# georgematheos/Gen

Measured on AMD Instinct MI355X. Metric: particle-steps/sec (whole node) + log-ML error vs CPU ref, 1M-particle SSM, higher is better.
Workload: dtype f64; 1 GPU; C2: 10-dim linear-Gaussian SSM bootstrap PF, 1048576 particles/GPU, systematic resampling at ESS<N/2, record_history=True; particles_global=1048576, d=10, resampler=systematic, parallelism=particle-dp1, transport=none, filters=46

## Files before the change

gen_amd/csrc/gh_kernels.h:

```cpp
#pragma once
#include "gh_models.h"

namespace gh {

constexpr int kBlock = 256;
constexpr int kScanItems = 4;
constexpr int kScanTile = kBlock * kScanItems;

constexpr int kTileP = 64;
__host__ __device__ __forceinline__ int64_t tbase(int64_t i, int D) { return (i >> 6) * (int64_t)(kTileP * D); }
__host__ __device__ __forceinline__ int64_t xidx(int64_t i, int k, int D) {
  const int l = (int)(i & 63);
  return tbase(i, D) + (k < (D & ~1) ? (k >> 1) * (2 * kTileP) + 2 * l + (k & 1) : (D - 1) * kTileP + l);
}
__host__ __device__ __forceinline__ int64_t slot_doubles(int64_t n, int D) {
  return ((n + kTileP - 1) / kTileP) * (int64_t)(kTileP * D);
}

struct DevScalars {
  double stats[3];
  double log_ml_est;
  double M, L, ess;
  double sM;
  uint64_t S;
  uint64_t base;
  uint64_t local;
  uint64_t o, Qs, Rs;
  double invN;
  double invS;
  int pending;
  int fire;
  int spend;
  int one;
  int error;
  unsigned ticket;
  unsigned ticket_q;
  unsigned ticket_c;
  double cM, cL, cess;
  int cfire, cerr;
  unsigned bar_gen;
  int64_t ra, rb;
  unsigned fire_streak;
};

constexpr int kErrBarrier = 7;
constexpr int kErrGenealogy = 7 | 1 << 8;
constexpr int kErrPeer = 7 | 2 << 8;

struct StepArgs {
  const double* xprev;
  int32_t* anc;
  const uint32_t* mark;
  const uint32_t* carry;
  uint32_t mark_idx;
  int mark_mode;
  int resampled;
  int buf;
  const double* remote;
  int64_t ld_remote;
  double* xout;
  double* logw;
  int64_t n;
  int64_t nvb;
  int max_only;
  int64_t lo;
  uint64_t seed;
  uint32_t t;
  int proposal;
  DevScalars* dev;
  double* pm;
  double* ps;
  double* ps2;
  double* stats_out;
  uint64_t* amax;
  int part;
  int64_t j0;
  int64_t vb_split, vb_skip;
  int64_t grid_blocks;
  double* rhist;
};

template <int CTRL, int ROW_MASK = 0xf>
__device__ __forceinline__ uint64_t dpp_u64(uint64_t v, uint64_t old) {
  const int lo = __builtin_amdgcn_update_dpp((int)(uint32_t)old, (int)(uint32_t)v, CTRL, ROW_MASK, 0xf, false);
  const int hi = __builtin_amdgcn_update_dpp((int)(uint32_t)(old >> 32), (int)(uint32_t)(v >> 32), CTRL, ROW_MASK,
                                             0xf, false);
  return ((uint64_t)(uint32_t)hi << 32) | (uint64_t)(uint32_t)lo;
}
template <int CTRL, int ROW_MASK = 0xf>
__device__ __forceinline__ double dpp_f64(double v, double old) {
  return as_f64(dpp_u64<CTRL, ROW_MASK>(as_u64(v), as_u64(old)));
}
__device__ __forceinline__ uint64_t readfirstlane_u64(uint64_t v) {
  const uint32_t lo = (uint32_t)__builtin_amdgcn_readfirstlane((int)(uint32_t)v);
  const uint32_t hi = (uint32_t)__builtin_amdgcn_readfirstlane((int)(uint32_t)(v >> 32));
  return ((uint64_t)hi << 32) | lo;
}
__device__ __forceinline__ uint64_t readlane63_u64(uint64_t v) {
  const uint32_t lo = (uint32_t)__builtin_amdgcn_readlane((int)(uint32_t)v, 63);
  const uint32_t hi = (uint32_t)__builtin_amdgcn_readlane((int)(uint32_t)(v >> 32), 63);
  return ((uint64_t)hi << 32) | lo;
}

template <int CTRL, int ROW_MASK = 0xf>
__device__ __forceinline__ uint64_t dpp_red_u64(uint64_t v) {
  const int lo = __builtin_amdgcn_mov_dpp((int)(uint32_t)v, CTRL, ROW_MASK, 0xf, true);
  const int hi = __builtin_amdgcn_mov_dpp((int)(uint32_t)(v >> 32), CTRL, ROW_MASK, 0xf, true);
  return ((uint64_t)(uint32_t)hi << 32) | (uint64_t)(uint32_t)lo;
}
template <int CTRL, int ROW_MASK = 0xf>
__device__ __forceinline__ double dpp_red_f64(double v) {
  return as_f64(dpp_red_u64<CTRL, ROW_MASK>(as_u64(v)));
}

template <class Op>
__device__ __forceinline__ double wave_reduce_f64(double v, Op op) {
  v = op(v, dpp_red_f64<0xb1>(v));
  v = op(v, dpp_red_f64<0x4e>(v));
  v = op(v, dpp_red_f64<0x114>(v));
  v = op(v, dpp_red_f64<0x118>(v));
  v = op(v, dpp_red_f64<0x142, 0xa>(v));
  v = op(v, dpp_red_f64<0x143, 0xc>(v));
  return as_f64(readlane63_u64(as_u64(v)));
}
__device__ __forceinline__ double wave_max(double v) {
  return wave_reduce_f64(v, [](double a, double b) { return fmax(a, b); });
}
__device__ __forceinline__ double wave_sum(double v) {
  return wave_reduce_f64(v, [](double a, double b) { return a + b; });
}
__device__ __forceinline__ uint64_t wave_sum_u64(uint64_t v) {
  v += dpp_red_u64<0xb1>(v);
  v += dpp_red_u64<0x4e>(v);
  v += dpp_red_u64<0x114>(v);
  v += dpp_red_u64<0x118>(v);
  v += dpp_red_u64<0x142, 0xa>(v);
  v += dpp_red_u64<0x143, 0xc>(v);
  return readlane63_u64(v);
}
__device__ __forceinline__ uint64_t wave_incl_sum_u64(uint64_t v) {
  v += dpp_u64<0x111>(v, 0);
  v += dpp_u64<0x112>(v, 0);
  v += dpp_u64<0x114>(v, 0);
  v += dpp_u64<0x118>(v, 0);
  v += dpp_u64<0x142, 0xa>(v, 0);
  v += dpp_u64<0x143, 0xc>(v, 0);
  return v;
}
template <int CTRL, int ROW_MASK = 0xf>
__device__ __forceinline__ uint32_t dpp0_u32(uint32_t v) {
  return (uint32_t)__builtin_amdgcn_update_dpp(0, (int)v, CTRL, ROW_MASK, 0xf, false);
}
__device__ __forceinline__ uint32_t wave_incl_max_u32(uint32_t v) {
  v = max(v, dpp0_u32<0x111>(v));
  v = max(v, dpp0_u32<0x112>(v));
  v = max(v, dpp0_u32<0x114>(v));
  v = max(v, dpp0_u32<0x118>(v));
  v = max(v, dpp0_u32<0x142, 0xa>(v));
  v = max(v, dpp0_u32<0x143, 0xc>(v));
  return v;
}
__device__ __forceinline__ uint64_t wave_incl_max_u64(uint64_t v) {
  const int lane = threadIdx.x & 63, rl = lane & 15;
  uint64_t t;
  t = dpp_u64<0x111>(v, 0); if (rl >= 1 && t > v) v = t;
  t = dpp_u64<0x112>(v, 0); if (rl >= 2 && t > v) v = t;
  t = dpp_u64<0x114>(v, 0); if (rl >= 4 && t > v) v = t;
  t = dpp_u64<0x118>(v, 0); if (rl >= 8 && t > v) v = t;
  t = dpp_u64<0x142>(v, 0); if ((lane & 31) >= 16 && t > v) v = t;
  t = dpp_u64<0x143>(v, 0); if (lane >= 32 && t > v) v = t;
  return v;
}

__device__ __forceinline__ double block_max(double v, double* sm) {
  v = wave_max(v);
  const int w = threadIdx.x >> 6;
  __syncthreads();
  if ((threadIdx.x & 63) == 0) sm[w] = v;
  __syncthreads();
  return fmax(fmax(sm[0], sm[1]), fmax(sm[2], sm[3]));
}
__device__ __forceinline__ double block_sum(double v, double* sm) {
  v = wave_sum(v);
  const int w = threadIdx.x >> 6;
  __syncthreads();
  if ((threadIdx.x & 63) == 0) sm[w] = v;
  __syncthreads();
  return (sm[0] + sm[1]) + (sm[2] + sm[3]);
}

template <class T>
__device__ __forceinline__ T ld_sc1(T* p) {
  return __hip_atomic_load(p, __ATOMIC_RELAXED, __HIP_MEMORY_SCOPE_AGENT);
}
template <class T>
__device__ __forceinline__ void st_sc1(T* p, T v) {
  __hip_atomic_store(p, v, __ATOMIC_RELAXED, __HIP_MEMORY_SCOPE_AGENT);
}

template <class T>
__device__ __forceinline__ T ld_sys(const T* p) {
  return __hip_atomic_load(const_cast<T*>(p), __ATOMIC_RELAXED, __HIP_MEMORY_SCOPE_SYSTEM);
}
template <class T>
__device__ __forceinline__ void st_sys(T* p, T v) {
  __hip_atomic_store(p, v, __ATOMIC_RELAXED, __HIP_MEMORY_SCOPE_SYSTEM);
}

typedef unsigned int gh_v2u __attribute__((ext_vector_type(2)));
__device__ __forceinline__ __amdgpu_buffer_rsrc_t gh_rsrc(const void* p) {
  return __builtin_amdgcn_make_buffer_rsrc(const_cast<void*>(p), 0, (int)0xffffffff, 0x00020000);
}
__device__ __forceinline__ double buf_ld_f64(__amdgpu_buffer_rsrc_t r, uint32_t voff, uint32_t soff) {
  return __builtin_bit_cast(double, __builtin_amdgcn_raw_buffer_load_b64(r, (int)voff, (int)soff, 0));
}
__device__ __forceinline__ void buf_st_f64(double v, __amdgpu_buffer_rsrc_t r, uint32_t voff, uint32_t soff) {
  __builtin_amdgcn_raw_buffer_store_b64(__builtin_bit_cast(gh_v2u, v), r, (int)voff, (int)soff, 0);
}
typedef unsigned int gh_v4u __attribute__((ext_vector_type(4)));
__device__ __forceinline__ void buf_ld_f64x2(__amdgpu_buffer_rsrc_t r, uint32_t voff, uint32_t soff, double* out) {
  const gh_v4u v = __builtin_amdgcn_raw_buffer_load_b128(r, (int)voff, (int)soff, 0);
  out[0] = __builtin_bit_cast(double, ((uint64_t)v.y << 32) | v.x);
  out[1] = __builtin_bit_cast(double, ((uint64_t)v.w << 32) | v.z);
}
__device__ __forceinline__ void buf_st_f64x2(const double* in, __amdgpu_buffer_rsrc_t r, uint32_t voff, uint32_t soff) {
  const uint64_t a = __builtin_bit_cast(uint64_t, in[0]), b = __builtin_bit_cast(uint64_t, in[1]);
  const gh_v4u v = {(unsigned)a, (unsigned)(a >> 32), (unsigned)b, (unsigned)(b >> 32)};
  __builtin_amdgcn_raw_buffer_store_b128(v, r, (int)voff, (int)soff, 0);
}

__device__ __forceinline__ void lds_barrier() { asm volatile("s_waitcnt lgkmcnt(0)\n\ts_barrier" ::: "memory"); }

__device__ __forceinline__ void block_partial(double lw, double (*sm)[4], double* pm, double* ps, double* ps2,
                                              int lane, int w, bool t0) {
  const double mw = wave_max(lw);
  if (lane == 0) sm[0][w] = mw;
  lds_barrier();
  const double mb = fmax(fmax(sm[0][0], sm[0][1]), fmax(sm[0][2], sm[0][3]));
  double e = 0.0;
  if (lw > -INFINITY) e = gh_exp_nonpos(lw - mb);
  if (lw != lw) e = lw;
  const double sw = wave_sum(e), s2w = wave_sum(e * e);
  if (lane == 0) {
    sm[1][w] = sw;
    sm[2][w] = s2w;
  }
  lds_barrier();
  if (t0) {
    *pm = mb;
    *ps = (sm[1][0] + sm[1][1]) + (sm[1][2] + sm[1][3]);
    *ps2 = (sm[2][0] + sm[2][1]) + (sm[2][2] + sm[2][3]);
  }
}
__device__ __forceinline__ void block_partial(double lw, double (*sm)[4], double* pm, double* ps, double* ps2) {
  block_partial(lw, sm, pm, ps, ps2, threadIdx.x & 63, threadIdx.x >> 6, threadIdx.x == 0);
}

constexpr int kAmaxShards = 32;
constexpr int kAmaxStride = 16;
constexpr uint64_t kAmaxEmpty = 0x000fffffffffffffull;
__host__ __device__ __forceinline__ uint64_t amax_key(double x) {
  const uint64_t b = x == x ? as_u64(x) : as_u64(-INFINITY);
  return (b >> 63) ? ~b : (b | 0x8000000000000000ull);
}
__host__ __device__ __forceinline__ double amax_value(uint64_t k) {
  return as_f64((k >> 63) ? (k & 0x7fffffffffffffffull) : ~k);
}

__device__ __forceinline__ void block_max_partial(double lw, double (*sm)[4], double* pm, uint64_t* amax,
                                                  int64_t vb, int lane, int w, bool t0) {
  const double mw = wave_max(lw);
  if (lane == 0) sm[0][w] = mw;
  lds_barrier();
  if (t0) {
    const double mb = fmax(fmax(sm[0][0], sm[0][1]), fmax(sm[0][2], sm[0][3]));
    *pm = mb;
    if (amax)
      __hip_atomic_fetch_max(&amax[(vb & (kAmaxShards - 1)) * kAmaxStride], amax_key(mb), __ATOMIC_RELAXED,
                             __HIP_MEMORY_SCOPE_AGENT);
  }
}
__device__ __forceinline__ void block_max_partial(double lw, double (*sm)[4], double* pm, uint64_t* amax,
                                                  int64_t vb) {
  block_max_partial(lw, sm, pm, amax, vb, threadIdx.x & 63, threadIdx.x >> 6, threadIdx.x == 0);
}

template <class M, class = void>
struct makes_calls : std::false_type {};
template <class M>
struct makes_calls<M, std::void_t<decltype(M::kCalls)>> : std::bool_constant<M::kCalls> {};
__device__ __forceinline__ int lane_now() {
  int l;
  asm volatile("v_mbcnt_lo_u32_b32 %0, -1, 0\n\tv_mbcnt_hi_u32_b32 %0, -1, %0" : "=v"(l));
  return l;
}

template <class Model, bool INIT, bool SPLIT = false>
__global__ __launch_bounds__(kBlock, Model::kMinWaves) void k_step(const double* __restrict__ prm,
                                                                    typename Model::Params p0, StepObs o,
                                                                    StepArgs a) {
  constexpr int D = Model::kD;
  const typename Model::Params p = p0.rebase(prm);
  __shared__ double sm[3][4];
  __shared__ double logtab[kMathTabDoubles];
  const int lane = threadIdx.x & 63, w = threadIdx.x >> 6;
  const int64_t vb = SPLIT ? (int64_t)blockIdx.x + (blockIdx.x >= a.vb_split ? a.vb_skip : 0) : (int64_t)blockIdx.x;
  const int ws = makes_calls<Model>::value ? __builtin_amdgcn_readfirstlane(w) : w;
  const int64_t tile = vb * (kBlock / 64) + w;
  const int64_t j = tile * 64 + lane;
  uint32_t mv = 0, cv = 0;
  int pending = 0, fire = 0;
  if (!INIT && a.resampled) {
    pending = a.dev->pending;
    fire = a.dev->fire;
    if (a.mark_mode) {
      const int64_t last = a.n > 0 ? a.n - 1 : 0;
      mv = a.mark[j < last ? j : last];
      cv = a.carry[tile < (last >> 6) ? tile : (last >> 6)];
    }
  }
  load_math_tab256(logtab);
  lds_barrier();
  asm volatile("" : "+v"(mv), "+v"(cv));
  const int pend = pending | fire;
  const int use_marks = a.mark_mode && fire && !pending;
  const Draw dr_init{STREAM_INIT, 0, logtab}, dr_step{STREAM_STEP, 0, logtab};
  double lw = -INFINITY;
  if (tile * 64 < a.n) {
    int64_t src = j;
    if (use_marks) {
      const uint32_t v = wave_incl_max_u32(max(j < a.n ? mv : 0u, cv));
      src = (int64_t)(v & a.mark_idx);
      if (a.mark_mode == 2) {
        const int64_t ra = a.dev->ra, rb = a.dev->rb, js = a.j0 + j;
        if (js < ra) src = -1 - js;
        else if (js >= rb) src = -1 - (ra + (js - rb));
      }
      if (j < a.n) a.anc[j] = (int32_t)src;
    }
    if (j < a.n && !(a.part == 1 && src < 0)) {
      double x[D];
      if (INIT) {
        lw = Model::init(p, o, a.seed, (uint64_t)(a.lo + j), a.proposal, x, dr_init);
      } else {
        double xp[D];
        if (pend && !use_marks) src = a.anc[j];
        if (a.buf && __builtin_amdgcn_ballot_w64(src < 0) == 0) {
          const __amdgpu_buffer_rsrc_t rp = gh_rsrc(a.xprev);
          const uint32_t tb = ((uint32_t)src >> 6) * (uint32_t)(kTileP * D * 8), l = (uint32_t)src & 63u;
#pragma unroll
          for (int c = 0; c < D / 2; ++c) buf_ld_f64x2(rp, tb + l * 16u, (uint32_t)(c * kTileP * 16), &xp[2 * c]);
          if (D & 1) xp[D - 1] = buf_ld_f64(rp, tb + l * 8u, (uint32_t)((D - 1) * kTileP * 8));
        } else {
          const bool loc = src >= 0;
#pragma unroll
          for (int k = 0; k < D; ++k)
            xp[k] = loc ? a.xprev[xidx(src, k, D)] : ld_sys(&a.remote[(-1 - src) * a.ld_remote + k]);
          if (SPLIT && !loc && a.rhist) {
            double* h = a.rhist + (-1 - src) * (int64_t)(D + 1);
#pragma unroll
            for (int k = 0; k < D; ++k) h[k] = xp[k];
            h[D] = ld_sys(&a.remote[(-1 - src) * a.ld_remote + D]);
          }
        }
        const double inc = Model::step(p, o, a.seed, (uint64_t)(a.lo + j), a.t, a.proposal, xp, x, dr_step);
        lw = (pend ? 0.0 : a.logw[j]) + inc;
      }

      if (a.buf) {
        const __amdgpu_buffer_rsrc_t ro = gh_rsrc(a.xout);
        const uint32_t tb = (uint32_t)tile * (uint32_t)(kTileP * D * 8);
#pragma unroll
        for (int c = 0; c < D / 2; ++c) buf_st_f64x2(&x[2 * c], ro, tb + (uint32_t)lane * 16u, (uint32_t)(c * kTileP * 16));
        if (D & 1) buf_st_f64(x[D - 1], ro, tb + (uint32_t)lane * 8u, (uint32_t)((D - 1) * kTileP * 8));
      } else {
#pragma unroll
        for (int k = 0; k < D; ++k) a.xout[xidx(j, k, D)] = x[k];
      }
      a.logw[j] = lw;
    }
  }
  if constexpr (makes_calls<Model>::value) {
    const int fl = lane_now();
    const bool t0 = fl == 0 && ws == 0;
    if (a.max_only) block_max_partial(lw, sm, a.pm + vb, a.amax, vb, fl, ws, t0);
    else block_partial(lw, sm, a.pm + vb, a.ps + vb, a.ps2 + vb, fl, ws, t0);
  } else {
    if (a.max_only) block_max_partial(lw, sm, a.pm + vb, a.amax, vb);
    else block_partial(lw, sm, a.pm + vb, a.ps + vb, a.ps2 + vb);
  }
}

__device__ __forceinline__ void block_partial2(double lw0, double lw1, double (*sm)[4], double* pm, double* ps,
                                               double* ps2) {
  const int lane = threadIdx.x & 63, w = threadIdx.x >> 6;
  const double mw = wave_max(fmax(lw0, lw1));
  if (lane == 0) sm[0][w] = mw;
  lds_barrier();
  const double mb = fmax(fmax(sm[0][0], sm[0][1]), fmax(sm[0][2], sm[0][3]));
  double e0 = 0.0, e1 = 0.0;
  if (lw0 > -INFINITY) e0 = gh_exp_nonpos(lw0 - mb);
  if (lw1 > -INFINITY) e1 = gh_exp_nonpos(lw1 - mb);
  if (lw0 != lw0) e0 = lw0;
  if (lw1 != lw1) e1 = lw1;
  const double sw = wave_sum(e0 + e1), s2w = wave_sum(e0 * e0 + e1 * e1);
  if (lane == 0) {
    sm[1][w] = sw;
    sm[2][w] = s2w;
  }
  lds_barrier();
  if (threadIdx.x == 0) {
    *pm = mb;
    *ps = (sm[1][0] + sm[1][1]) + (sm[1][2] + sm[1][3]);
    *ps2 = (sm[2][0] + sm[2][1]) + (sm[2][2] + sm[2][3]);
  }
}

template <class Model, bool INIT, bool SPLIT = false>
__global__ __launch_bounds__(kBlock, Model::kMinWaves) void k_step_pairs(const double* __restrict__ prm,
                                                                          typename Model::Params p0, StepObs o,
                                                                          StepArgs a) {
  static_assert(Model::kD == 1 && Model::kPairs, "pair stepping: one-dimensional paired models");
  const typename Model::Params p = p0.rebase(prm);
  __shared__ double sm[3][4];
  __shared__ double logtab[kMathTabDoubles];
  const int lane = threadIdx.x & 63, w = threadIdx.x >> 6;
  const int64_t vb = SPLIT ? (int64_t)blockIdx.x + (blockIdx.x >= a.vb_split ? a.vb_skip : 0) : (int64_t)blockIdx.x;
  const int64_t tile0 = (vb * (kBlock / 64) + w) * 2;
  const int64_t j0 = tile0 * 64 + lane, j1 = j0 + 64;
  uint32_t mv0 = 0, mv1 = 0, cv0 = 0, cv1 = 0;
  int pending = 0, fire = 0;
  if (!INIT && a.resampled) {
    pending = a.dev->pending;
    fire = a.dev->fire;
    if (a.mark_mode) {
      const int64_t last = a.n > 0 ? a.n - 1 : 0, lt = last >> 6;
      mv0 = a.mark[j0 < last ? j0 : last];
      mv1 = a.mark[j1 < last ? j1 : last];
      cv0 = a.carry[tile0 < lt ? tile0 : lt];
      cv1 = a.carry[tile0 + 1 < lt ? tile0 + 1 : lt];
    }
  }
  load_math_tab256(logtab);
  lds_barrier();
  asm volatile("" : "+v"(mv0), "+v"(cv0), "+v"(mv1), "+v"(cv1));
  const int pend = pending | fire;
  const int use_marks = a.mark_mode && fire && !pending;
  const Draw dr_init{STREAM_INIT, 0, logtab}, dr_step{STREAM_STEP, 0, logtab};
  double lw0 = -INFINITY, lw1 = -INFINITY;
  if (tile0 * 64 < a.n) {
    const bool has1 = j1 < a.n;
    int64_t s0 = j0, s1 = j1;
    if (use_marks) {
      const uint32_t v0 = wave_incl_max_u32(max(j0 < a.n ? mv0 : 0u, cv0));
      const uint32_t v1 = wave_incl_max_u32(max(has1 ? mv1 : 0u, cv1));
      s0 = (int64_t)(v0 & a.mark_idx);
      s1 = (int64_t)(v1 & a.mark_idx);
      if (a.mark_mode == 2) {
        const int64_t ra = a.dev->ra, rb = a.dev->rb, js0 = a.j0 + j0, js1 = a.j0 + j1;
        if (js0 < ra) s0 = -1 - js0;
        else if (js0 >= rb) s0 = -1 - (ra + (js0 - rb));
        if (js1 < ra) s1 = -1 - js1;
        else if (js1 >= rb) s1 = -1 - (ra + (js1 - rb));
      }
      if (j0 < a.n) a.anc[j0] = (int32_t)s0;
      if (has1) a.anc[j1] = (int32_t)s1;
    }
    if (j0 < a.n) {
      const uint64_t g0 = (uint64_t)(a.lo + j0);
      double x0, x1, w0, w1;
      bool skip0 = false, skip1 = false;
      if (INIT) {
        Model::init2(p, o, a.seed, g0, &x0, &x1, &w0, &w1, dr_init);
      } else {
        if (pend && !use_marks) {
          s0 = a.anc[j0];
          s1 = has1 ? a.anc[j1] : s0;
        }
        if (!has1) s1 = s0;
        double xp0, xp1;
        if (a.remote && __builtin_amdgcn_ballot_w64(s0 < 0 || s1 < 0) != 0) {
          skip0 = a.part == 1 && s0 < 0;
          skip1 = a.part == 1 && s1 < 0;
          xp0 = s0 >= 0 ? a.xprev[s0] : (skip0 ? 0.0 : ld_sys(&a.remote[(-1 - s0) * a.ld_remote]));
          xp1 = s1 >= 0 ? a.xprev[s1] : (skip1 ? 0.0 : ld_sys(&a.remote[(-1 - s1) * a.ld_remote]));
          if (SPLIT && a.rhist) {
            if (s0 < 0) {
              a.rhist[(-1 - s0) * 2] = xp0;
              a.rhist[(-1 - s0) * 2 + 1] = ld_sys(&a.remote[(-1 - s0) * a.ld_remote + 1]);
            }
            if (has1 && s1 < 0) {
              a.rhist[(-1 - s1) * 2] = xp1;
              a.rhist[(-1 - s1) * 2 + 1] = ld_sys(&a.remote[(-1 - s1) * a.ld_remote + 1]);
            }
          }
        } else {
          xp0 = a.xprev[s0];
          xp1 = a.xprev[s1];
        }
        Model::step2(p, o, a.seed, g0, a.t, xp0, xp1, &x0, &x1, &w0, &w1, dr_step);
        w0 = (pend ? 0.0 : a.logw[j0]) + w0;
        if (has1) w1 = (pend ? 0.0 : a.logw[j1]) + w1;
      }
      if (!skip0) {
        a.xout[j0] = x0;
        a.logw[j0] = w0;
        lw0 = w0;
      }
      if (has1 && !skip1) {
        a.xout[j1] = x1;
        a.logw[j1] = w1;
        lw1 = w1;
      }
    }
  }
  if (a.max_only) block_max_partial(fmax(lw0, lw1), sm, a.pm + vb, a.amax, vb);
  else block_partial2(lw0, lw1, sm, a.pm + vb, a.ps + vb, a.ps2 + vb);
}

template <bool PAIRS>
__global__ __launch_bounds__(kBlock) void k_block_sums(const double* __restrict__ logw, int64_t n,
                                                        const double* __restrict__ pm, double* ps, double* ps2) {
  __shared__ double sm[2][4];
  const int lane = threadIdx.x & 63, w = threadIdx.x >> 6;
  const int64_t vb = blockIdx.x;
  const double mb = pm[vb];
  double sw, s2w;
  if (!PAIRS) {
    const int64_t j = (vb * (kBlock / 64) + w) * 64 + lane;
    const double lw = j < n ? logw[j] : -INFINITY;
    double e = 0.0;
    if (lw > -INFINITY) e = gh_exp_nonpos(lw - mb);
    if (lw != lw) e = lw;
    sw = wave_sum(e);
    s2w = wave_sum(e * e);
  } else {
    const int64_t j0 = (vb * (kBlock / 64) + w) * 2 * 64 + lane, j1 = j0 + 64;
    const double lw0 = j0 < n ? logw[j0] : -INFINITY, lw1 = j1 < n ? logw[j1] : -INFINITY;
    double e0 = 0.0, e1 = 0.0;
    if (lw0 > -INFINITY) e0 = gh_exp_nonpos(lw0 - mb);
    if (lw1 > -INFINITY) e1 = gh_exp_nonpos(lw1 - mb);
    if (lw0 != lw0) e0 = lw0;
    if (lw1 != lw1) e1 = lw1;
    sw = wave_sum(e0 + e1);
    s2w = wave_sum(e0 * e0 + e1 * e1);
  }
  if (lane == 0) {
    sm[0][w] = sw;
    sm[1][w] = s2w;
  }
  lds_barrier();
  if (threadIdx.x == 0) {
    ps[vb] = (sm[0][0] + sm[0][1]) + (sm[0][2] + sm[0][3]);
    ps2[vb] = (sm[1][0] + sm[1][1]) + (sm[1][2] + sm[1][3]);
  }
}

struct DecideArgs {
  const double* stats_all;
  int R;
  int64_t n_global;
  double log_n;
  double inv_n;
  double thr;
  double* ess_hist;
  int32_t* res_hist;
  int t;
};

struct Decision {
  double M, L, ess;
  int fire, err;
};

__device__ __forceinline__ Decision decide(const DecideArgs& d, bool uniform) {
  Decision r{};
  double M = -INFINITY;
  if (uniform) M = 0.0;
  else
    for (int q = 0; q < d.R; ++q) M = fmax(M, d.stats_all[3 * q]);
  if (!(M > -INFINITY) || M == INFINITY || M != M) {
    r.err = 3;
    r.ess = NAN;
    r.M = M;
    return r;
  }
  double S = 0.0, S2 = 0.0;
  for (int q = 0; q < d.R; ++q) {
    if (uniform) {
      const double nq = (double)((d.n_global * (q + 1)) / d.R - (d.n_global * q) / d.R);
      S += nq * 1.0;
      S2 += nq * 1.0;
      continue;
    }
    if (!(d.stats_all[3 * q] > -INFINITY)) continue;
    const double e = gh_exp(d.stats_all[3 * q] - M);
    S += d.stats_all[3 * q + 1] * e;
    S2 += d.stats_all[3 * q + 2] * (e * e);
  }
  r.M = M;
  r.L = M + gh_log(S);
  r.ess = (S * S) / S2;
  r.fire = r.ess < d.thr;
  return r;
}

__device__ __forceinline__ void commit_decision(const DecideArgs& d, const Decision& r, DevScalars* dev,
                                                int pending) {
  dev->M = r.M;
  dev->L = r.L;
  dev->ess = r.ess;
  dev->fire = r.fire;
  if (r.err) dev->error = r.err;
  if (r.fire) dev->log_ml_est += r.L - d.log_n;
  if (d.ess_hist) d.ess_hist[d.t] = r.ess;
  if (d.res_hist) d.res_hist[d.t + 1] = pending | r.fire;
}

static __global__ void k_decide(DecideArgs d, DevScalars* dev) {
  if (threadIdx.x != 0 || blockIdx.x != 0) return;
  if (dev->fire) {
    dev->pending = 1;
    dev->fire = 0;
  }
  const Decision r = decide(d, dev->pending != 0);
  commit_decision(d, r, dev, dev->pending);
}

static __global__ __launch_bounds__(1024) void k_fold(const double* pm, const double* ps, const double* ps2, int nb,
                                               double* stats_out, DevScalars* dev, int clear_flags,
                                               double thr_hint, int64_t n_global) {
  __shared__ double sm[16];
  const int lane = threadIdx.x & 63, w = threadIdx.x >> 6;
  double m = -INFINITY;
  for (int b0 = threadIdx.x; b0 < nb; b0 += 1024 * 8) {
    double v[8];
#pragma unroll
    for (int k = 0; k < 8; ++k) v[k] = (b0 + 1024 * k < nb) ? pm[b0 + 1024 * k] : -INFINITY;
#pragma unroll
    for (int k = 0; k < 8; ++k) m = fmax(m, v[k]);
  }
  m = wave_max(m);
  if (lane == 0) sm[w] = m;
  __syncthreads();
  double M = -INFINITY;
  for (int k = 0; k < 16; ++k) M = fmax(M, sm[k]);
// ... 1675 lines not shown
```

gen_amd/csrc/gh_models.h:

```cpp
#pragma once
#include "gh_math.h"

namespace gh {

constexpr int kMaxObs = 32;

struct Draw {
  uint32_t stream;
  uint32_t base;
  const double* tab = nullptr;
};

struct StepObs {
  double v[kMaxObs];
  double ct;
  int present;
  int sym;
};

template <class P>
__device__ __forceinline__ const double* rebased(const P& p, const double* __restrict__ prm, const double* ptr) {
  return prm + (ptr - p.base);
}

struct LGParams {
  const double* base;
  const double* A;
  const double* b;
  const double* LQ;
  const double* M;
  const double* mu0;
  const double* L0;
  const double* FA;
  const double* LSig;
  const double* WA;
  const double* LSig1;
  const double* H;
  const double* cv;
  const double* LR;
  const double* QP = nullptr;
  const double* QL = nullptr;
  double cstq = 0.0;
  int dy;
  double cstR;
  double cstS;
  double cstQ, cst0;
  __device__ LGParams rebase(const double* __restrict__ prm) const {
    LGParams q = *this;
    q.A = rebased(*this, prm, A);
    q.b = rebased(*this, prm, b);
    q.LQ = rebased(*this, prm, LQ);
    q.M = rebased(*this, prm, M);
    q.mu0 = rebased(*this, prm, mu0);
    q.L0 = rebased(*this, prm, L0);
    q.FA = rebased(*this, prm, FA);
    q.LSig = rebased(*this, prm, LSig);
    q.WA = rebased(*this, prm, WA);
    q.LSig1 = rebased(*this, prm, LSig1);
    q.H = rebased(*this, prm, H);
    q.cv = rebased(*this, prm, cv);
    q.LR = rebased(*this, prm, LR);
    return q;
  }
};

template <int D, int S = 0>
struct LGModel {
  static constexpr int kD = D;
  #if defined(GH_LG10_WAVES)
  static constexpr int kMinWaves = (D <= 4) ? 8 : (D <= 10 ? (S == 3 ? GH_LG10_WAVES : 5) : 4);
#else
  static constexpr int kMinWaves =
      (D <= 3) ? 8 : (D <= 5 ? 7 : (D < 10 ? (S == 3 && D != 7 && D != 9 ? 6 : 5) : (D == 10 ? (S == 3 ? 7 : 5) : 4)));
#endif
  using Params = LGParams;

  __device__ static double obs(const Params& p, const StepObs& o, const double* x) {
    if (!o.present) return 0.0;
    double quad = 0.0;
    if (S & 2) {
#pragma unroll
      for (int r = 0; r < D; ++r) {
        const double acc = fma(-p.M[r * D + r], x[r], o.v[r]);
        quad = fma(acc, acc, quad);
      }
    } else {
      for (int r = 0; r < p.dy; ++r) {
        double acc = o.v[r];
#pragma unroll
        for (int j = 0; j < D; ++j) acc = fma(-p.M[r * D + j], x[j], acc);
        quad = fma(acc, acc, quad);
      }
    }
    return p.cstR - 0.5 * quad;
  }

  __device__ static double loglik(const Params& p, const StepObs& o, const double* x) { return obs(p, o, x); }

  __device__ static void score(const Params& p, const StepObs& o, uint32_t t, const double* xp, const double* x,
                               double* lat, double* ob) {
    const double* L = t == 1 ? p.L0 : p.LQ;
    double u[D];
    double quad = 0.0;
#pragma unroll
    for (int i = 0; i < D; ++i) {
      double mean;
      if (t == 1) {
        mean = p.mu0[i];
      } else {
        mean = p.b[i];
#pragma unroll
        for (int k = 0; k < D; ++k) mean = fma(p.A[i * D + k], xp[k], mean);
      }
      double r = x[i] - mean;
      if (t == 1 || !(S & 1)) {
#pragma unroll
        for (int k = 0; k < i; ++k) r = fma(-L[i * D + k], u[k], r);
      }
      u[i] = r / L[i * D + i];
      quad = fma(u[i], u[i], quad);
    }
    *lat = (t == 1 ? p.cst0 : p.cstQ) - 0.5 * quad;
    *ob = obs(p, o, x);
  }

  __device__ static double sim_obs(const Params& p, uint64_t seed, uint64_t pid, uint32_t t, const double* x,
                                   double* y, int64_t ys, const double* tab) {
    double z[kMaxObs], v[kMaxObs];
    normals_rt(seed, pid, t, STREAM_SIM, kSimObsDraw, p.dy, z, tab);
    for (int r = 0; r < p.dy; ++r) {
      double acc = p.cv[r];
#pragma unroll
      for (int j = 0; j < D; ++j) acc = fma(p.H[r * D + j], x[j], acc);
      for (int k = 0; k <= r; ++k) acc = fma(p.LR[r * p.dy + k], z[k], acc);
      y[r * ys] = acc;
      double s = acc - p.cv[r];
      for (int k = 0; k < r; ++k) s = fma(-p.LR[r * p.dy + k], v[k], s);
      v[r] = s / p.LR[r * p.dy + r];
    }
    double quad = 0.0;
    if (S & 2) {
#pragma unroll
      for (int r = 0; r < D; ++r) {
        const double acc = fma(-p.M[r * D + r], x[r], v[r]);
        quad = fma(acc, acc, quad);
      }
    } else {
      for (int r = 0; r < p.dy; ++r) {
        double acc = v[r];
#pragma unroll
        for (int j = 0; j < D; ++j) acc = fma(-p.M[r * D + j], x[j], acc);
        quad = fma(acc, acc, quad);
      }
    }
    return p.cstR - 0.5 * quad;
  }

  __device__ static double init(const Params& p, const StepObs& o, uint64_t seed, uint64_t pid,
                                int , double* x, Draw dr = {STREAM_INIT, 0}) {
    double z[D + 1];
    normals_n<D>(seed, pid, 1, dr.stream, dr.base, z, dr.tab);
#pragma unroll
    for (int i = 0; i < D; ++i) {
      double acc = p.mu0[i];
#pragma unroll
      for (int k = 0; k <= i; ++k) acc = fma(p.L0[i * D + k], z[k], acc);
      x[i] = acc;
    }
    return obs(p, o, x);
  }

  __device__ static double step(const Params& p, const StepObs& o, uint64_t seed, uint64_t pid,
                                uint32_t t, int , const double* xp, double* x,
                                Draw dr = {STREAM_STEP, 0}) {
    double z[D + 1];
    normals_n<D>(seed, pid, t, dr.stream, dr.base, z, dr.tab);
#pragma unroll
    for (int i = 0; i < D; ++i) {
      double acc = p.b[i];
#pragma unroll
      for (int k = 0; k < D; ++k) acc = fma(p.A[i * D + k], xp[k], acc);
      if (S & 1) {
        acc = fma(p.LQ[i * D + i], z[i], acc);
      } else {
#pragma unroll
        for (int k = 0; k <= i; ++k) acc = fma(p.LQ[i * D + k], z[k], acc);
      }
      x[i] = acc;
    }
    return obs(p, o, x);
  }
};

template <int D>
struct LGOptModel {
  static constexpr int kD = D;
  static constexpr int kMinWaves = (D <= 4) ? 8 : (D <= 8 ? 5 : (D <= 14 ? 4 : 3));
  using Params = LGParams;
  using Prior = LGModel<D, 0>;

  __device__ static double loglik(const Params& p, const StepObs& o, const double* x) { return Prior::loglik(p, o, x); }

  __device__ static double init(const Params& p, const StepObs& o, uint64_t seed, uint64_t pid, int proposal,
                                double* x, Draw dr = {STREAM_INIT, 0}) {
    if (!o.present) return Prior::init(p, o, seed, pid, proposal, x, dr);
    double z[D + 1];
    normals_n<D>(seed, pid, 1, dr.stream, dr.base, z, dr.tab);
#pragma unroll
    for (int i = 0; i < D; ++i) {
      double acc = o.v[i];
#pragma unroll
      for (int k = 0; k <= i; ++k) acc = fma(p.LSig1[i * D + k], z[k], acc);
      x[i] = acc;
    }
    return o.ct;
  }

  __device__ static double step(const Params& p, const StepObs& o, uint64_t seed, uint64_t pid, uint32_t t,
                                int proposal, const double* xp, double* x, Draw dr = {STREAM_STEP, 0}) {
    if (!o.present) return Prior::step(p, o, seed, pid, t, proposal, xp, x, dr);
    double z[D + 1];
    normals_n<D>(seed, pid, t, dr.stream, dr.base, z, dr.tab);
#pragma unroll
    for (int i = 0; i < D; ++i) {
      double acc = o.v[i];
#pragma unroll
      for (int k = 0; k < D; ++k) acc = fma(p.FA[i * D + k], xp[k], acc);
#pragma unroll
      for (int k = 0; k <= i; ++k) acc = fma(p.LSig[i * D + k], z[k], acc);
      x[i] = acc;
    }
    double quad = 0.0;
    for (int r = 0; r < p.dy; ++r) {
      double u = o.v[D + r];
#pragma unroll
      for (int k = 0; k < D; ++k) u = fma(-p.WA[r * D + k], xp[k], u);
      quad = fma(u, u, quad);
    }
    return p.cstS - 0.5 * quad;
  }
};

template <int D>
struct LGLinModel {
  static constexpr int kD = D;
  static constexpr int kMinWaves = (D <= 4) ? 8 : (D <= 8 ? 5 : (D <= 14 ? 4 : 3));
  using Params = LGParams;
  using Prior = LGModel<D, 0>;

  __device__ static double loglik(const Params& p, const StepObs& o, const double* x) { return Prior::loglik(p, o, x); }

  __device__ static double draw(const Params& p, const StepObs& o, const double* xp, const double* z, double* x) {
#pragma unroll
    for (int i = 0; i < D; ++i) {
      double acc = o.v[p.dy + i];
      if (xp) {
#pragma unroll
        for (int k = 0; k < D; ++k) acc = fma(p.QP[i * D + k], xp[k], acc);
      }
#pragma unroll
      for (int k = 0; k <= i; ++k) acc = fma(p.QL[i * D + k], z[k], acc);
      x[i] = acc;
    }
    double w[D];
    double quad = 0.0;
#pragma unroll
    for (int i = 0; i < D; ++i) {
      double mean = o.v[p.dy + i];
      if (xp) {
#pragma unroll
        for (int k = 0; k < D; ++k) mean = fma(p.QP[i * D + k], xp[k], mean);
      }
      double r = x[i] - mean;
#pragma unroll
      for (int k = 0; k < i; ++k) r = fma(-p.QL[i * D + k], w[k], r);
      w[i] = r / p.QL[i * D + i];
      quad = fma(w[i], w[i], quad);
    }
    return p.cstq - 0.5 * quad;
  }

  __device__ static double init(const Params& p, const StepObs& o, uint64_t seed, uint64_t pid, int ,
                                double* x, Draw dr = {STREAM_INIT, 0}) {
    double z[D + 1];
    normals_n<D>(seed, pid, 1, dr.stream, dr.base, z, dr.tab);
    const double lq = draw(p, o, nullptr, z, x);
    double lat, ob;
    Prior::score(p, o, 1, x, x, &lat, &ob);
    return (lat + ob) - lq;
  }

  __device__ static double step(const Params& p, const StepObs& o, uint64_t seed, uint64_t pid, uint32_t t,
                                int , const double* xp, double* x, Draw dr = {STREAM_STEP, 0}) {
    double z[D + 1];
    normals_n<D>(seed, pid, t, dr.stream, dr.base, z, dr.tab);
    const double lq = draw(p, o, xp, z, x);
    double lat, ob;
    Prior::score(p, o, t, xp, x, &lat, &ob);
    return (lat + ob) - lq;
  }
};

struct HMMParams {
  const double* base;
  const double* prior;
  const double* T;
  const double* E;
  const double* logE;
  int k;
  int v;
  __device__ HMMParams rebase(const double* __restrict__ prm) const {
    HMMParams q = *this;
    q.prior = rebased(*this, prm, prior);
    q.T = rebased(*this, prm, T);
    q.E = rebased(*this, prm, E);
    q.logE = rebased(*this, prm, logE);
    return q;
  }
};

__device__ __forceinline__ int cat_sample(const double* p, int K, int stride, double u) {
  double total = 0.0;
  for (int k = 0; k < K; ++k) total += p[k * stride];
  const double target = u * total;
  double cum = 0.0;
  int last = -1;
  for (int k = 0; k < K; ++k) {
    const double pk = p[k * stride];
    cum += pk;
    if (pk > 0.0) last = k;
    if (cum > target && pk > 0.0) return k;
  }
  return last;
}

__device__ __forceinline__ int cat_sample_prod(const double* a, int sa, const double* e, int K,
                                               double u, double* total_out) {
  double total = 0.0;
  for (int k = 0; k < K; ++k) total += a[k * sa] * e[k];
  *total_out = total;
  const double target = u * total;
  double cum = 0.0;
  int last = -1;
  for (int k = 0; k < K; ++k) {
    const double pk = a[k * sa] * e[k];
    cum += pk;
    if (pk > 0.0) last = k;
    if (cum > target && pk > 0.0) return k;
  }
  return last;
}

struct HMMModel {
  static constexpr int kD = 1;
  static constexpr int kMinWaves = 8;
  using Params = HMMParams;

  __device__ static double loglik(const Params& p, const StepObs& o, const double* x) {
    return o.present ? p.logE[o.sym * p.k + (int)x[0]] : 0.0;
  }
  __device__ static void score(const Params& p, const StepObs& o, uint32_t t, const double* xp, const double* x,
                               double* lat, double* ob) {
    const int z = (int)x[0];
    *lat = gh_log(t == 1 ? p.prior[z] : p.T[z * p.k + (int)xp[0]]);
    *ob = loglik(p, o, x);
  }
  __device__ static double sim_obs(const Params& p, uint64_t seed, uint64_t pid, uint32_t t, const double* x,
                                   double* y, int64_t, const double*) {
    const int z = (int)x[0];
    const u32x4 w = rng_block(seed, pid, t, STREAM_SIM, kSimObsDraw);
    const int sym = cat_sample(p.E + z, p.v, p.k, u53(w.x, w.y));
    y[0] = (double)sym;
    return p.logE[sym * p.k + z];
  }
  __device__ static double init(const Params& p, const StepObs& o, uint64_t seed, uint64_t pid,
                                int proposal, double* x, Draw dr = {STREAM_INIT, 0}) {
    const u32x4 w = rng_block(seed, pid, 1, dr.stream, dr.base);
    const double u = u53(w.x, w.y);
    if (proposal == 1 && o.present) {
      double total;
      const int z = cat_sample_prod(p.prior, 1, p.E + o.sym * p.k, p.k, u, &total);
      x[0] = (double)z;
      return gh_log(total);
    }
    const int z = cat_sample(p.prior, p.k, 1, u);
    x[0] = (double)z;
    return o.present ? p.logE[o.sym * p.k + z] : 0.0;
  }

  __device__ static double step(const Params& p, const StepObs& o, uint64_t seed, uint64_t pid,
                                uint32_t t, int proposal, const double* xp, double* x,
                                Draw dr = {STREAM_STEP, 0}) {
    const u32x4 w = rng_block(seed, pid, t, dr.stream, dr.base);
    const double u = u53(w.x, w.y);
    const int zp = (int)xp[0];
    if (proposal == 1 && o.present) {
      double total;
      const int z = cat_sample_prod(p.T + zp, p.k, p.E + o.sym * p.k, p.k, u, &total);
      x[0] = (double)z;
      return gh_log(total);
    }
    const int z = cat_sample(p.T + zp, p.k, p.k, u);
    x[0] = (double)z;
    return o.present ? p.logE[o.sym * p.k + z] : 0.0;
  }
};

struct KitParams {
  double mu1, s1;
  double sx;
  double inv2vy;
  double csty;
  double inv2vx, cstx;
  double inv2v1, cst1;
  double sy;
  __device__ KitParams rebase(const double* __restrict__) const { return *this; }
};

__device__ __forceinline__ uint64_t kit_pair_id(uint64_t pid) { return ((pid >> 7) << 6) | (pid & 63); }

struct KitModel {
  static constexpr int kD = 1;
  static constexpr int kMinWaves = 8;
  static constexpr bool kPairs = true;
  using Params = KitParams;

  __device__ static double obs(const Params& p, const StepObs& o, double x) {
    if (!o.present) return 0.0;
    const double diff = o.v[0] - div20(x * x);
    return -(diff * diff) * p.inv2vy + p.csty;
  }
  __device__ static double loglik(const Params& p, const StepObs& o, const double* x) { return obs(p, o, x[0]); }
  __device__ static void score(const Params& p, const StepObs& o, uint32_t t, const double* xp, const double* x,
                               double* lat, double* ob) {
    double mean = p.mu1, inv2 = p.inv2v1, cst = p.cst1;
    if (t > 1) {
      const double v = xp[0];
      mean = ((v / 2.0) + 25.0 * (v / (1.0 + v * v))) + o.ct;
      inv2 = p.inv2vx;
      cst = p.cstx;
    }
    const double d = x[0] - mean;
    *lat = -(d * d) * inv2 + cst;
    *ob = obs(p, o, x[0]);
  }
  __device__ static double sim_obs(const Params& p, uint64_t seed, uint64_t pid, uint32_t t, const double* x,
                                   double* y, int64_t, const double* tab) {
    double z0, z1;
    normal_pair(rng_block(seed, pid, t, STREAM_SIM, kSimObsDraw), &z0, &z1, tab);
    const double m = div20(x[0] * x[0]);
    y[0] = m + p.sy * z0;
    const double diff = y[0] - m;
    return -(diff * diff) * p.inv2vy + p.csty;
  }
  __device__ static double mean(const StepObs& o, double v) { return ((v / 2.0) + 25.0 * (v / (1.0 + v * v))) + o.ct; }
  __device__ static double znorm(uint64_t seed, uint64_t pid, uint32_t t, const Draw& dr) {
    double z0, z1;
    normal_pair(rng_block(seed, kit_pair_id(pid), t, dr.stream, dr.base), &z0, &z1, dr.tab);
    return ((pid >> 6) & 1) ? z1 : z0;
  }
  __device__ static double init(const Params& p, const StepObs& o, uint64_t seed, uint64_t pid,
                                int , double* x, Draw dr = {STREAM_INIT, 0}) {
    x[0] = p.mu1 + p.s1 * znorm(seed, pid, 1, dr);
    return obs(p, o, x[0]);
  }
  __device__ static double step(const Params& p, const StepObs& o, uint64_t seed, uint64_t pid,
                                uint32_t t, int , const double* xp, double* x,
                                Draw dr = {STREAM_STEP, 0}) {
    x[0] = mean(o, xp[0]) + p.sx * znorm(seed, pid, t, dr);
    return obs(p, o, x[0]);
  }
  __device__ static void init2(const Params& p, const StepObs& o, uint64_t seed, uint64_t pid0, double* x0,
                               double* x1, double* w0, double* w1, const Draw& dr) {
    double z0, z1;
    normal_pair(rng_block(seed, kit_pair_id(pid0), 1, dr.stream, dr.base), &z0, &z1, dr.tab);
    *x0 = p.mu1 + p.s1 * z0;
    *x1 = p.mu1 + p.s1 * z1;
    *w0 = obs(p, o, *x0);
    *w1 = obs(p, o, *x1);
// ... 114 lines not shown
```

Baseline: 20.71 billion particle-steps/s.

## Stage ancestor state pairs through LDS via buffer-load-to-LDS in LG10 step

```diff
diff --git a/gen_amd/csrc/gh_kernels.h b/gen_amd/csrc/gh_kernels.h
--- a/gen_amd/csrc/gh_kernels.h
+++ b/gen_amd/csrc/gh_kernels.h
@@ -229,6 +229,27 @@
   __builtin_amdgcn_raw_buffer_store_b128(v, r, (int)voff, (int)soff, 0);
 }
 
+template <int IMM>
+__device__ __forceinline__ void buf_ld_lds_f64x2(__amdgpu_buffer_rsrc_t r, uint32_t voff, void* lds) {
+  __builtin_amdgcn_raw_ptr_buffer_load_lds(r, (__attribute__((address_space(3))) void*)lds, 16, (int)voff, 0, IMM, 0);
+}
+template <int P, int C = 0>
+__device__ __forceinline__ void stage_pairs(__amdgpu_buffer_rsrc_t r, uint32_t voff, void* lds) {
+  if constexpr (C < P) {
+    buf_ld_lds_f64x2<C * kTileP * 16>(r, voff, lds);
+    stage_pairs<P, C + 1>(r, voff, lds);
+  }
+}
+
+template <class M, class = void>
+struct lds_pairs : std::integral_constant<int, 0> {};
+template <class M>
+struct lds_pairs<M, std::void_t<decltype(M::kLdsPairs)>> : std::integral_constant<int, M::kLdsPairs> {};
+template <class M, bool INIT, bool SPLIT, class = void>
+struct step_waves : std::integral_constant<int, M::kMinWaves> {};
+template <class M>
+struct step_waves<M, false, false, std::void_t<decltype(M::kStepWaves)>> : std::integral_constant<int, M::kStepWaves> {};
+
 __device__ __forceinline__ void lds_barrier() { asm volatile("s_waitcnt lgkmcnt(0)\n\ts_barrier" ::: "memory"); }
 
 __device__ __forceinline__ void block_partial(double lw, double (*sm)[4], double* pm, double* ps, double* ps2,
@@ -296,10 +317,11 @@
 }
 
 template <class Model, bool INIT, bool SPLIT = false>
-__global__ __launch_bounds__(kBlock, Model::kMinWaves) void k_step(const double* __restrict__ prm,
-                                                                    typename Model::Params p0, StepObs o,
-                                                                    StepArgs a) {
+__global__ __launch_bounds__(kBlock, (step_waves<Model, INIT, SPLIT>::value)) void k_step(
+    const double* __restrict__ prm, typename Model::Params p0, StepObs o, StepArgs a) {
   constexpr int D = Model::kD;
+  constexpr int P = (INIT || SPLIT) ? 0 : lds_pairs<Model>::value;
+  static_assert(P <= D / 2, "kLdsPairs counts whole component pairs");
   const typename Model::Params p = p0.rebase(prm);
   __shared__ double sm[3][4];
   __shared__ double logtab[kMathTabDoubles];
@@ -342,6 +364,32 @@
       double x[D];
       if (INIT) {
         lw = Model::init(p, o, a.seed, (uint64_t)(a.lo + j), a.proposal, x, dr_init);
+      } else if constexpr (P > 0) {
+        __shared__ gh_v4u xstage[kBlock / 64][P][kTileP];
+        gh_v4u* const st = &xstage[w][0][0];
+        StagedPrev<D, P> xs;
+        xs.lds = reinterpret_cast<const double*>(st + lane);
+        if (pend && !use_marks) src = a.anc[j];
+        if (a.buf && __builtin_amdgcn_ballot_w64(src < 0) == 0) {
+          const __amdgpu_buffer_rsrc_t rp = gh_rsrc(a.xprev);
+          const uint32_t tb = ((uint32_t)src >> 6) * (uint32_t)(kTileP * D * 8), l = (uint32_t)src & 63u;
+          stage_pairs<P>(rp, tb + l * 16u, st);
+#pragma unroll
+          for (int c = P; c < D / 2; ++c) buf_ld_f64x2(rp, tb + l * 16u, (uint32_t)(c * kTileP * 16), &xs.r[2 * c]);
+          if (D & 1) xs.r[D - 1] = buf_ld_f64(rp, tb + l * 8u, (uint32_t)((D - 1) * kTileP * 8));
+        } else {
+          const bool loc = src >= 0;
+#pragma unroll
+          for (int k = 0; k < D; ++k)
+            xs.r[k] = loc ? a.xprev[xidx(src, k, D)] : ld_sys(&a.remote[(-1 - src) * a.ld_remote + k]);
+#pragma unroll
+          for (int c = 0; c < P; ++c) {
+            const uint64_t u = as_u64(xs.r[2 * c]), v = as_u64(xs.r[2 * c + 1]);
+            st[c * kTileP + lane] = gh_v4u{(unsigned)u, (unsigned)(u >> 32), (unsigned)v, (unsigned)(v >> 32)};
+          }
+        }
+        const double inc = Model::step(p, o, a.seed, (uint64_t)(a.lo + j), a.t, a.proposal, xs, x, dr_step);
+        lw = (pend ? 0.0 : a.logw[j]) + inc;
       } else {
         double xp[D];
         if (pend && !use_marks) src = a.anc[j];
diff --git a/gen_amd/csrc/gh_models.h b/gen_amd/csrc/gh_models.h
--- a/gen_amd/csrc/gh_models.h
+++ b/gen_amd/csrc/gh_models.h
@@ -64,6 +64,27 @@
   }
 };
 
+template <int D, int P>
+struct StagedPrev {
+  const double* lds;
+  double r[D];
+  __device__ __forceinline__ void get(double* xp) const {
+    asm volatile("s_waitcnt vmcnt(0)" ::: "memory");
+#pragma unroll
+    for (int c = 0; c < P; ++c) {
+      const double2 v = *reinterpret_cast<const double2*>(lds + c * 128);
+      xp[2 * c] = v.x;
+      xp[2 * c + 1] = v.y;
+    }
+#pragma unroll
+    for (int k = 2 * P; k < D; ++k) xp[k] = r[k];
+  }
+};
+
+#if !defined(GH_LG10_LDS_PAIRS)
+#define GH_LG10_LDS_PAIRS 3
+#endif
+
 template <int D, int S = 0>
 struct LGModel {
   static constexpr int kD = D;
@@ -73,6 +94,12 @@
   static constexpr int kMinWaves =
       (D <= 3) ? 8 : (D <= 5 ? 7 : (D < 10 ? (S == 3 && D != 7 && D != 9 ? 6 : 5) : (D == 10 ? (S == 3 ? 7 : 5) : 4)));
 #endif
+  static constexpr int kLdsPairs = (D == 10 && S == 3) ? GH_LG10_LDS_PAIRS : 0;
+#if defined(GH_LG10_WAVES)
+  static constexpr int kStepWaves = kMinWaves;
+#else
+  static constexpr int kStepWaves = kLdsPairs > 0 ? 8 : kMinWaves;
+#endif
   using Params = LGParams;
 
   __device__ static double obs(const Params& p, const StepObs& o, const double* x) {
@@ -175,6 +202,22 @@
                                 Draw dr = {STREAM_STEP, 0}) {
     double z[D + 1];
     normals_n<D>(seed, pid, t, dr.stream, dr.base, z, dr.tab);
+    return step_mean_noise(p, o, xp, z, x);
+  }
+
+  template <int P>
+  __device__ static double step(const Params& p, const StepObs& o, uint64_t seed, uint64_t pid,
+                                uint32_t t, int , const StagedPrev<D, P>& xs, double* x,
+                                Draw dr = {STREAM_STEP, 0}) {
+    double z[D + 1];
+    normals_n<D>(seed, pid, t, dr.stream, dr.base, z, dr.tab);
+    double xp[D];
+    xs.get(xp);
+    return step_mean_noise(p, o, xp, z, x);
+  }
+
+  __device__ __forceinline__ static double step_mean_noise(const Params& p, const StepObs& o, const double* xp,
+                                                           const double* z, double* x) {
 #pragma unroll
     for (int i = 0; i < D; ++i) {
       double acc = p.b[i];
```

New measurement: 21.20 billion particle-steps/s (median of 6 runs). 2.4% higher.
